# microsoft/ANCE

Measured on NVIDIA H100. Metric: ANN-refresh throughput: passages encoded/sec + queries top-200/sec, 8.8M x 768, higher is better.
Workload: dtype fp16

## Files before the change

### ance_b200/csrc/gemm_core.cuh

```cuda
#pragma once
#include "tc05.cuh"

namespace gemm {

using namespace tc05;

constexpr int BM = 128;
constexpr int BK = 64;
constexpr int MMA_K = 16;

struct WorkShape {
  int M, N, K;
  int num_m_blks;
  int num_n_blks;
  int n_splits;
  int n_blks_per_split;
  unsigned long long hint_a, hint_b;
  int* pace;
  int pace_window;
  int pace_stride;
};

static __device__ __noinline__ void pace_wait(int* pace, int window, int me, int n_clusters, int stride, int seq) {
  volatile int* vp = pace;
  vp[me] = seq;
  const long long t0 = clock64();
  for (;;) {
    int mn = 0x7fffffff;
    for (int c = me % stride; c < n_clusters; c += stride) mn = min(mn, vp[c]);
    if (seq - mn <= window || clock64() - t0 > 200000ll) break;
  }
}

struct EpiCtx {
  int m_blk, split;
  int nb0, nb1;
  int row0;
  int quad;
  int epi_warp;
  int lane;
  int work_seq;
  uint8_t* ep_smem;
};

template <int BN, int STAGES, int CG, int EP_SMEM = 0>
struct SmemPlan {
  static constexpr int kABytes = BM * BK * 2;
  static constexpr int kBBytes = BN * BK * 2;
  static constexpr int kBHalfRows = BN / CG;
  static constexpr int kStageBytes = kABytes + kBBytes;
  static constexpr int kRingBytes = STAGES * kStageBytes;
  static constexpr int kAccPitch = BN + 4;
  static constexpr int kAccOffset = kRingBytes;
  static constexpr int kAccBytes = (BM * kAccPitch * 4 + 1023) / 1024 * 1024;
  static constexpr int kEpOffset = kAccOffset + kAccBytes;
  static constexpr int kBarOffset = kEpOffset + EP_SMEM;
  static constexpr int kBarBytes = (2 * STAGES + 2) * 8;
  static constexpr int kTotal = kBarOffset + kBarBytes;
  static constexpr int kDynamicBytes = kTotal + 1024;
  static_assert(kDynamicBytes <= 232448, "GEMM shared memory exceeds 227 KB");
};

template <uint32_t FMT, int BN>
__device__ __forceinline__ void wgmma_tile(float (&d)[BN / 2], uint64_t adesc, uint64_t bdesc, uint32_t accumulate) {
  if constexpr (BN == 128) wgmma_n128<FMT, 0>(d, adesc, bdesc, accumulate);
  else wgmma_n64<FMT, 0>(d, adesc, bdesc, accumulate);
}

template <class Ep, int BN, int STAGES, int CG, int EPI_WARPS, uint32_t FMT>
__global__ void __launch_bounds__(256 + 32 * EPI_WARPS, 1)
tc05_gemm_kernel(const __grid_constant__ CUtensorMap tmA, const __grid_constant__ CUtensorMap tmB,
                 const WorkShape ws, const __grid_constant__ typename Ep::Params ep) {
  static_assert(BN == 64 || BN == 128, "BN");
  static_assert(CG == 1 || CG == 2, "CG");
  using Plan = SmemPlan<BN, STAGES, CG, Ep::kSmemBytes>;

  extern __shared__ uint8_t smem_raw[];
  uint8_t* smem = reinterpret_cast<uint8_t*>((reinterpret_cast<uintptr_t>(smem_raw) + 1023) & ~uintptr_t(1023));
  float* acc_tile = reinterpret_cast<float*>(smem + Plan::kAccOffset);
  uint64_t* full_bar = reinterpret_cast<uint64_t*>(smem + Plan::kBarOffset);
  uint64_t* empty_bar = full_bar + STAGES;
  uint64_t* afull_bar = empty_bar + STAGES;
  uint64_t* aempty_bar = afull_bar + 1;

  const int warp = threadIdx.x >> 5;
  const int lane = threadIdx.x & 31;
  const uint32_t cta_rank = (CG == 2) ? cluster_ctarank() : 0u;
  const bool leader = (cta_rank == 0);
  const int cluster_id = (CG == 2) ? (blockIdx.x >> 1) : blockIdx.x;
  const int num_clusters = (CG == 2) ? (gridDim.x >> 1) : gridDim.x;
  const int total_work = ws.num_m_blks * ws.n_splits;
  const int num_kb = (ws.K + BK - 1) / BK;

  if (warp == 0 && lane == 0) {
    tma_prefetch_desc(&tmA);
    tma_prefetch_desc(&tmB);
    for (int s = 0; s < STAGES; ++s) {
      mbar_init(&full_bar[s], 1);
      mbar_init(&empty_bar[s], 4 * CG);
    }
    mbar_init(afull_bar, 4);
    mbar_init(aempty_bar, EPI_WARPS);
    fence_barrier_init();
  }
  if constexpr (CG == 2) cluster_sync_all(); else __syncthreads();

  if (warp == 0) {
    if (lane == 0) {
      const uint64_t hint_a = ws.hint_a ? ws.hint_a : Ep::kHintA, hint_b = ws.hint_b ? ws.hint_b : Ep::kHintB;
      Ring<STAGES> ring;
      for (int w = cluster_id; w < total_work; w += num_clusters) {
        const int m_blk = w / ws.n_splits, split = w - m_blk * ws.n_splits;
        const int nb0 = split * ws.n_blks_per_split;
        const int nb1 = min(nb0 + ws.n_blks_per_split, ws.num_n_blks);
        const int a_row = (m_blk * CG + (int)cta_rank) * BM;
        for (int nb = nb0; nb < nb1; ++nb) {
          if (ws.pace != nullptr && leader && ((nb - nb0) & 7) == 0)
            pace_wait(ws.pace, ws.pace_window, cluster_id, num_clusters, ws.pace_stride,
                      ((w - cluster_id) / num_clusters) * ws.num_n_blks + (nb - nb0));
          const int b_row = nb * BN + (int)cta_rank * Plan::kBHalfRows;
          for (int kb = 0; kb < num_kb; ++kb) {
            mbar_wait(&empty_bar[ring.stage], ring.phase ^ 1, 1);
            uint8_t* sa = smem + ring.stage * Plan::kStageBytes;
            uint8_t* sb = sa + Plan::kABytes + cta_rank * (Plan::kBHalfRows * 128);
            mbar_arrive_expect_tx(&full_bar[ring.stage], Plan::kStageBytes);
            tma_load_2d(sa, &tmA, &full_bar[ring.stage], kb * BK, a_row, hint_a);
            if constexpr (CG == 1) tma_load_2d(sb, &tmB, &full_bar[ring.stage], kb * BK, b_row, hint_b);
            else tma_load_2d_multicast(sb, &tmB, &full_bar[ring.stage], kb * BK, b_row, 0x3, hint_b);
            ring.advance();
          }
        }
      }
      if (ws.pace != nullptr && leader) *reinterpret_cast<volatile int*>(ws.pace + cluster_id) = 0x7fffffff;
    }
  } else if (warp >= 4 && warp < 8) {
    Ring<STAGES> ring;
    uint32_t acc_phase = 0;
    auto release = [&](int stage) {
      __syncwarp();
      if (lane == 0) {
        mbar_arrive(&empty_bar[stage]);
        if constexpr (CG == 2) mbar_arrive_cluster(&empty_bar[stage], cta_rank ^ 1u);
      }
    };
    for (int w = cluster_id; w < total_work; w += num_clusters) {
      const int m_blk = w / ws.n_splits, split = w - m_blk * ws.n_splits;
      const int nb0 = split * ws.n_blks_per_split;
      const int nb1 = min(nb0 + ws.n_blks_per_split, ws.num_n_blks);
      (void)m_blk;
      for (int nb = nb0; nb < nb1; ++nb) {
        float acc0[BN / 2], acc1[BN / 2];
#pragma unroll
        for (int i = 0; i < BN / 2; ++i) acc0[i] = acc1[i] = 0.f;
        int prev_stage = -1;
        for (int kb = 0; kb < num_kb; ++kb) {
          mbar_wait(&full_bar[ring.stage], ring.phase, 3);
          const uint32_t sa = smem_u32(smem + ring.stage * Plan::kStageBytes);
          const uint32_t sb = sa + Plan::kABytes;
          wgmma_fence();
#pragma unroll
          for (int k = 0; k < BK / MMA_K; ++k) {
            const uint64_t bdesc = make_desc_k_sw128(sb + k * MMA_K * 2);
            wgmma_tile<FMT, BN>(acc0, make_desc_k_sw128(sa + k * MMA_K * 2), bdesc, 1u);
            wgmma_tile<FMT, BN>(acc1, make_desc_k_sw128(sa + 64 * 128 + k * MMA_K * 2), bdesc, 1u);
          }
          wgmma_commit();
          wgmma_wait<1>();
          wgmma_fence_regs(acc0);
          wgmma_fence_regs(acc1);
          if (prev_stage >= 0) release(prev_stage);
          prev_stage = ring.stage;
          ring.advance();
        }
        wgmma_wait<0>();
        wgmma_fence_regs(acc0);
        wgmma_fence_regs(acc1);
        if (prev_stage >= 0) release(prev_stage);
        mbar_wait(aempty_bar, acc_phase ^ 1, 2);
        acc_store_frag(acc_tile, Plan::kAccPitch, 0, 0, acc0);
        acc_store_frag(acc_tile, Plan::kAccPitch, 64, 0, acc1);
        __syncwarp();
        if (lane == 0) mbar_arrive(afull_bar);
        acc_phase ^= 1;
      }
    }
  } else if (warp >= 8) {
    Ep epi;
    EpiCtx cx;
    cx.quad = warp & 3;
    cx.epi_warp = warp - 8;
    cx.lane = lane;
    cx.work_seq = 0;
    cx.ep_smem = smem + Plan::kEpOffset;
    uint32_t acc_phase = 0;
    const uint32_t tacc = smem_u32(acc_tile) / 4u + static_cast<uint32_t>((cx.quad * 32 + lane) * Plan::kAccPitch);
    for (int w = cluster_id; w < total_work; w += num_clusters, ++cx.work_seq) {
      cx.m_blk = w / ws.n_splits;
      cx.split = w - cx.m_blk * ws.n_splits;
      cx.nb0 = cx.split * ws.n_blks_per_split;
      cx.nb1 = min(cx.nb0 + ws.n_blks_per_split, ws.num_n_blks);
      cx.row0 = (cx.m_blk * CG + (int)cta_rank) * BM;
      epi.begin_work(ep, ws, cx);
      for (int nb = cx.nb0; nb < cx.nb1; ++nb) {
        mbar_wait(afull_bar, acc_phase, 4);
        epi.tile(ep, ws, cx, tacc, nb);
        __syncwarp();
        if (lane == 0) mbar_arrive(aempty_bar);
        acc_phase ^= 1;
      }
      epi.end_work(ep, ws, cx);
    }
    epi.end_kernel(ep, cx);
  }

  if constexpr (CG == 2) cluster_sync_all();
}

constexpr int kMaxDevices = 64;

inline int current_device() {
  int dev = 0;
  cudaGetDevice(&dev);
  return (dev >= 0 && dev < kMaxDevices) ? dev : 0;
}

inline int sm_count() {
  static int n[kMaxDevices] = {};
  const int dev = current_device();
  if (!n[dev]) cudaDeviceGetAttribute(&n[dev], cudaDevAttrMultiProcessorCount, dev);
  return n[dev];
}

template <class Ep, int BN, int STAGES, int CG, int EPI_WARPS, uint32_t FMT>
cudaError_t launch(const CUtensorMap& tmA, const CUtensorMap& tmB, const WorkShape& ws,
                   const typename Ep::Params& ep, int max_ctas, cudaStream_t stream) {
  using Plan = SmemPlan<BN, STAGES, CG, Ep::kSmemBytes>;
  auto kern = tc05_gemm_kernel<Ep, BN, STAGES, CG, EPI_WARPS, FMT>;
  static bool configured[kMaxDevices] = {};
  const int dev = current_device();
  if (!configured[dev]) {
    cudaError_t e = cudaFuncSetAttribute(kern, cudaFuncAttributeMaxDynamicSharedMemorySize, Plan::kDynamicBytes);
    if (e != cudaSuccess) return e;
    configured[dev] = true;
  }
  const int total = ws.num_m_blks * ws.n_splits;
  int clusters = min(total, (max_ctas > 0 ? max_ctas : sm_count()) / CG);
  if (clusters < 1) clusters = 1;
  cudaLaunchConfig_t cfg = {};
  cfg.gridDim = dim3(clusters * CG);
  cfg.blockDim = dim3(256 + 32 * EPI_WARPS);
  cfg.dynamicSmemBytes = Plan::kDynamicBytes;
  cfg.stream = stream;
  cudaLaunchAttribute attr[1];
  attr[0].id = cudaLaunchAttributeClusterDimension;
  attr[0].val.clusterDim.x = CG;
  attr[0].val.clusterDim.y = 1;
  attr[0].val.clusterDim.z = 1;
  cfg.attrs = attr;
  cfg.numAttrs = 1;
  return cudaLaunchKernelEx(&cfg, kern, tmA, tmB, ws, ep);
}

inline WorkShape make_shape(int M, int N, int K, int BN, int CG, int n_splits ) {
  WorkShape ws;
  ws.M = M;
  ws.N = N;
  ws.K = K;
  ws.num_m_blks = (M + BM * CG - 1) / (BM * CG);
  ws.num_n_blks = (N + BN - 1) / BN;
  if (n_splits <= 0 || n_splits > ws.num_n_blks) n_splits = ws.num_n_blks;
  ws.n_blks_per_split = (ws.num_n_blks + n_splits - 1) / n_splits;
  ws.n_splits = (ws.num_n_blks + ws.n_blks_per_split - 1) / ws.n_blks_per_split;
  ws.hint_a = ws.hint_b = 0;
  ws.pace = nullptr;
  ws.pace_window = 0;
  ws.pace_stride = 1;
  return ws;
}

}
```

### ance_b200/csrc/gemm_store.cuh

```cuda
#pragma once
#include "act16.cuh"
#include "gemm_core.cuh"

namespace gemm {

__device__ __forceinline__ float rcp_approx(float x) {
  float r;
  asm("rcp.approx.ftz.f32 %0, %1;" : "=f"(r) : "f"(x));
  return r;
}
__device__ __forceinline__ float ex2_approx(float x) {
  float r;
  asm("ex2.approx.ftz.f32 %0, %1;" : "=f"(r) : "f"(x));
  return r;
}

__device__ __forceinline__ uint64_t pack2(float a, float b) {
  uint64_t r;
  asm("mov.b64 %0, {%1, %2};" : "=l"(r) : "f"(a), "f"(b));
  return r;
}
__device__ __forceinline__ void unpack2(uint64_t v, float& a, float& b) {
  asm("mov.b64 {%0, %1}, %2;" : "=f"(a), "=f"(b) : "l"(v));
}
__device__ __forceinline__ uint64_t fma2(uint64_t a, uint64_t b, uint64_t c) {
  float a0, a1, b0, b1, c0, c1;
  unpack2(a, a0, a1), unpack2(b, b0, b1), unpack2(c, c0, c1);
  return pack2(__fmaf_rn(a0, b0, c0), __fmaf_rn(a1, b1, c1));
}
__device__ __forceinline__ uint64_t mul2(uint64_t a, uint64_t b) {
  float a0, a1, b0, b1;
  unpack2(a, a0, a1), unpack2(b, b0, b1);
  return pack2(__fmul_rn(a0, b0), __fmul_rn(a1, b1));
}

__device__ __forceinline__ void gelu_erf2(float& x0, float& x1) {
  const uint64_t x = pack2(x0, x1);
  const uint64_t ax = x & 0x7FFFFFFF7FFFFFFFull;
  uint64_t p = fma2(pack2(5.38297490e-06f, 5.38297490e-06f), ax, pack2(4.88906371e-05f, 4.88906371e-05f));
  p = fma2(p, ax, pack2(3.80035744e-05f, 3.80035744e-05f));
  p = fma2(p, ax, pack2(3.27762635e-03f, 3.27762635e-03f));
  p = fma2(p, ax, pack2(2.11410057e-02f, 2.11410057e-02f));
  p = fma2(p, ax, pack2(4.98673469e-02f, 4.98673469e-02f));
  p = fma2(p, ax, pack2(1.0f, 1.0f));
  p = mul2(p, p);
  p = mul2(p, p);
  p = mul2(p, p);
  p = mul2(p, p);
  float p0, p1;
  unpack2(p, p0, p1);
  const uint64_t r = pack2(rcp_approx(p0), rcp_approx(p1));
  const uint64_t relu = fma2(ax, pack2(0.5f, 0.5f), mul2(x, pack2(0.5f, 0.5f)));
  unpack2(fma2(mul2(ax, pack2(-0.5f, -0.5f)), r, relu), x0, x1);
}

__device__ __forceinline__ void gelu_logistic2(float& x0, float& x1) {
  const uint64_t x = pack2(x0, x1);
  const uint64_t t = mul2(x, x);
  uint64_t p = fma2(pack2(-3.290565928e-06f, -3.290565928e-06f), t, pack2(8.930850163e-05f, 8.930850163e-05f));
  p = fma2(p, t, pack2(3.548454260e-04f, 3.548454260e-04f));
  p = fma2(p, t, pack2(-1.052178442e-01f, -1.052178442e-01f));
  p = fma2(p, t, pack2(-2.302048445e+00f, -2.302048445e+00f));
  float g0, g1;
  unpack2(mul2(p, x), g0, g1);
  const uint64_t d = fma2(pack2(ex2_approx(g0), ex2_approx(g1)), pack2(1.0f, 1.0f), pack2(1.0f, 1.0f));
  float d0, d1;
  unpack2(d, d0, d1);
  unpack2(mul2(x, pack2(rcp_approx(d0), rcp_approx(d1))), x0, x1);
}

template <int BN, int EPI_WARPS, uint32_t FMT = tc05::kFmtBF16>
struct EpStore {
  using A16 = act16::Act<FMT>;
  static constexpr uint64_t kHintA = tc05::kEvictNormal;
  static constexpr uint64_t kHintB = tc05::kEvictLast;
  static constexpr int kColGroups = EPI_WARPS / 4;
  static constexpr int kColsPerGroup = BN / kColGroups;
  static constexpr int kSlabBytes = BM * 128;
  static constexpr int kSmemBytes = kColGroups * kSlabBytes + 64;
  static_assert(EPI_WARPS % 4 == 0 && kColsPerGroup % 64 == 0, "epilogue warp layout");

  struct alignas(64) Params {
    CUtensorMap tmC;
    CUtensorMap tmR;
    uint16_t* C;
    float* C32;
    const float* bias;
    const uint16_t* R;
    int ldc, ldc32, ldr;
    int act;
  };

  uint32_t rphase;

  __device__ __forceinline__ void begin_work(const Params& p, const WorkShape&, const EpiCtx& cx) {
    if (cx.work_seq == 0 && p.R && p.C && !p.C32) {
      const int cgi = cx.epi_warp >> 2;
      uint64_t* rbar = reinterpret_cast<uint64_t*>(cx.ep_smem + kColGroups * kSlabBytes) + cgi;
      if ((cx.epi_warp & 3) == 0 && cx.lane == 0) {
        tc05::mbar_init(rbar, 1);
        tc05::fence_barrier_init();
      }
      tc05::named_bar_sync(2 + cgi, 128);
      rphase = 0;
    }
  }
  __device__ __forceinline__ void end_work(const Params&, const WorkShape&, const EpiCtx&) {}
  __device__ __forceinline__ void end_kernel(const Params& p, const EpiCtx& cx) {
    if (p.C && (cx.epi_warp & 3) == 0 && cx.lane == 0) tc05::bulk_wait_all();
  }

  __device__ __forceinline__ void finish_chunk(const Params& p, const WorkShape& ws, float (&f)[32], int row,
                                               bool row_ok, int col0, bool direct_residual) {
    const bool full = (col0 + 32 <= ws.N);
    if (p.bias) {
      if (full) {
#pragma unroll
        for (int j = 0; j < 8; ++j) {
          const float4 b = __ldg(reinterpret_cast<const float4*>(p.bias + col0) + j);
          f[j * 4] += b.x; f[j * 4 + 1] += b.y; f[j * 4 + 2] += b.z; f[j * 4 + 3] += b.w;
        }
      } else {
#pragma unroll
        for (int i = 0; i < 32; ++i)
          if (col0 + i < ws.N) f[i] += __ldg(p.bias + col0 + i);
      }
    }
    if (p.act == 1) {
#pragma unroll
      for (int i = 0; i < 32; i += 2) gelu_erf2(f[i], f[i + 1]);
    } else if (p.act == 2) {
#pragma unroll
      for (int i = 0; i < 32; i += 2) gelu_logistic2(f[i], f[i + 1]);
    }
    if (direct_residual && p.R && row_ok) {
      const uint16_t* r = p.R + (size_t)row * p.ldr + col0;
      if (full) {
#pragma unroll
        for (int j = 0; j < 4; ++j) {
          const uint4 q = __ldg(reinterpret_cast<const uint4*>(r) + j);
          const uint32_t h[4] = {q.x, q.y, q.z, q.w};
#pragma unroll
          for (int t = 0; t < 4; ++t) {
            const float2 x = A16::unpack2(h[t]);
            f[j * 8 + t * 2] += x.x;
            f[j * 8 + t * 2 + 1] += x.y;
          }
        }
      } else {
        for (int i = 0; i < 32; ++i)
          if (col0 + i < ws.N) f[i] += A16::to_float(r[i]);
      }
    }
  }

  __device__ __forceinline__ void tile(const Params& p, const WorkShape& ws, const EpiCtx& cx, uint32_t tacc,
                                       int nb) {
    const int cgi = cx.epi_warp >> 2;
    const int r_in_tile = cx.quad * 32 + cx.lane;
    const int row = cx.row0 + r_in_tile;
    const bool row_ok = row < ws.M;
    uint8_t* slab = cx.ep_smem + cgi * kSlabBytes;
    const bool issuer = (cx.epi_warp & 3) == 0 && cx.lane == 0;
#pragma unroll 1
    for (int s = 0; s < kColsPerGroup; s += 64) {
      const int col_in_tile = cgi * kColsPerGroup + s;
      const int col0 = nb * BN + col_in_tile;
      if (col0 >= ws.N) break;
      const bool tma_res = (p.R != nullptr) && (p.C != nullptr) && (p.C32 == nullptr);
      uint64_t* rbar = reinterpret_cast<uint64_t*>(cx.ep_smem + kColGroups * kSlabBytes) + cgi;
      uint8_t* rowp = slab + r_in_tile * 128;
      if (tma_res && issuer) {
        tc05::bulk_wait_read_all();
        tc05::mbar_arrive_expect_tx(rbar, kSlabBytes);
        tc05::tma_load_2d(slab, &p.tmR, rbar, col0, cx.row0, tc05::kEvictFirst);
      }
      constexpr bool kLean = EPI_WARPS > 8;
      uint32_t va[32], vb[kLean ? 1 : 32];
      tc05::acc_ld_x32(tacc + col_in_tile, va);
      if constexpr (!kLean) tc05::acc_ld_x32(tacc + col_in_tile + 32, vb);
      if (!tma_res && p.C) {
        if (issuer) tc05::bulk_wait_read_all();
        tc05::named_bar_sync(2 + cgi, 128);
      }
#pragma unroll
      for (int h = 0; h < 2; ++h) {
        float f[32];
        if constexpr (kLean) {
          if (h == 1) {
            tc05::acc_ld_x32(tacc + col_in_tile + 32, va);
          }
#pragma unroll
          for (int i = 0; i < 32; ++i) f[i] = __uint_as_float(va[i]);
        } else {
#pragma unroll
          for (int i = 0; i < 32; ++i) f[i] = __uint_as_float(h == 0 ? va[i] : vb[i]);
        }
        finish_chunk(p, ws, f, row, row_ok, col0 + h * 32, !tma_res);
        if (p.C32 && row_ok) {
          float* o = p.C32 + (size_t)row * p.ldc32 + col0 + h * 32;
          if (col0 + h * 32 + 32 <= ws.N) {
#pragma unroll
            for (int j = 0; j < 8; ++j)
              reinterpret_cast<float4*>(o)[j] = make_float4(f[j * 4], f[j * 4 + 1], f[j * 4 + 2], f[j * 4 + 3]);
          } else {
            for (int i = 0; i < 32; ++i)
              if (col0 + h * 32 + i < ws.N) o[i] = f[i];
          }
        }
        if (p.C) {
          if (tma_res && h == 0) tc05::mbar_wait(rbar, rphase, 20);
#pragma unroll
          for (int q = 0; q < 4; ++q) {
            uint4* cp = reinterpret_cast<uint4*>(rowp + (((h * 4 + q) ^ (r_in_tile & 7)) * 16));
            if (tma_res) {
              const uint4 rv = *cp;
              const uint32_t rh[4] = {rv.x, rv.y, rv.z, rv.w};
#pragma unroll
              for (int t = 0; t < 4; ++t) {
                const float2 x = A16::unpack2(rh[t]);
                f[q * 8 + t * 2] += x.x;
                f[q * 8 + t * 2 + 1] += x.y;
              }
            }
            uint4 o;
            o.x = A16::pack2(f[q * 8 + 0], f[q * 8 + 1]);
            o.y = A16::pack2(f[q * 8 + 2], f[q * 8 + 3]);
            o.z = A16::pack2(f[q * 8 + 4], f[q * 8 + 5]);
            o.w = A16::pack2(f[q * 8 + 6], f[q * 8 + 7]);
            *cp = o;
          }
        }
      }
      if (p.C) {
        if (tma_res) rphase ^= 1;
        tc05::fence_proxy_async_smem();
        tc05::named_bar_sync(2 + cgi, 128);
        if (issuer) {
          tc05::tma_store_2d(&p.tmC, slab, col0, cx.row0);
          tc05::bulk_commit_group();
        }
      }
    }
  }
};

inline bool make_store_tmap(CUtensorMap* tm, void* C, int M, int N, int ldc) {
  return tc05_host::make_tmap_2d_16b(tm, C, M, N, ldc, BM, 64);
}

}
```

### ance_b200/csrc/search.cu

```cuda
#include <float.h>
#include <math.h>
#include <string.h>

#include <algorithm>
#include <vector>

#include "common.h"
#include "gemm_core.cuh"

namespace {

using namespace tc05;

__host__ __device__ __forceinline__ uint32_t f2ord(float f) {
#ifdef __CUDA_ARCH__
  uint32_t u = __float_as_uint(f);
#else
  uint32_t u;
  memcpy(&u, &f, 4);
#endif
  return u ^ (static_cast<uint32_t>(static_cast<int32_t>(u) >> 31) | 0x80000000u);
}
__host__ __device__ __forceinline__ float ord2f(uint32_t k) {
  uint32_t u = (k & 0x80000000u) ? (k ^ 0x80000000u) : ~k;
#ifdef __CUDA_ARCH__
  return __uint_as_float(u);
#else
  float f;
  memcpy(&f, &u, 4);
  return f;
#endif
}
__device__ __forceinline__ uint64_t make_key(float score, uint32_t row) {
  return (static_cast<uint64_t>(f2ord(score)) << 32) | static_cast<uint64_t>(0xFFFFFFFFu - row);
}
__device__ __forceinline__ float key_score(uint64_t k) { return ord2f(static_cast<uint32_t>(k >> 32)); }
__device__ __forceinline__ uint32_t key_row(uint64_t k) { return 0xFFFFFFFFu - static_cast<uint32_t>(k); }

template <class T>
__device__ __forceinline__ T* shfl_ptr(T* p, int src) {
  uint64_t v = reinterpret_cast<uint64_t>(p);
  uint32_t lo = __shfl_sync(0xffffffffu, static_cast<uint32_t>(v), src);
  uint32_t hi = __shfl_sync(0xffffffffu, static_cast<uint32_t>(v >> 32), src);
  return reinterpret_cast<T*>((static_cast<uint64_t>(hi) << 32) | lo);
}

template <bool kBF16>
__global__ void quantize_rows_kernel(const float* __restrict__ X, uint16_t* __restrict__ X16, int64_t n, int d,
                                     const float* __restrict__ mu, float* __restrict__ norm_hat,
                                     float* __restrict__ norm_delta, unsigned int* __restrict__ max_stats,
                                     int* __restrict__ err_flag) {
  const int lane = threadIdx.x & 31;
  const int64_t row = static_cast<int64_t>(blockIdx.x) * (blockDim.x >> 5) + (threadIdx.x >> 5);
  if (row >= n) return;
  const float* x = X + row * d;
  uint16_t* o = X16 + row * d;
  float sh = 0.f, sd = 0.f, sx = 0.f;
  bool bad = false;
  for (int i = lane * 4; i < d; i += 128) {
    float4 v = __ldg(reinterpret_cast<const float4*>(x + i));
    if (mu) {
      const float4 m = __ldg(reinterpret_cast<const float4*>(mu + i));
      v.x -= m.x; v.y -= m.y; v.z -= m.z; v.w -= m.w;
    }
    float a[4] = {v.x, v.y, v.z, v.w};
    uint16_t q[4];
#pragma unroll
    for (int t = 0; t < 4; ++t) {
      float back;
      if (kBF16) {
        __nv_bfloat16 h = __float2bfloat16_rn(a[t]);
        q[t] = __bfloat16_as_ushort(h);
        back = __bfloat162float(h);
      } else {
        __half h = __float2half_rn(a[t]);
        q[t] = __half_as_ushort(h);
        back = __half2float(h);
      }
      if (!(fabsf(back) <= 3.0e38f)) bad = true;
      sh = fmaf(back, back, sh);
      const float e = a[t] - back;
      sd = fmaf(e, e, sd);
      sx = fmaf(a[t], a[t], sx);
    }
    uint2 pk;
    pk.x = static_cast<uint32_t>(q[0]) | (static_cast<uint32_t>(q[1]) << 16);
    pk.y = static_cast<uint32_t>(q[2]) | (static_cast<uint32_t>(q[3]) << 16);
    *reinterpret_cast<uint2*>(o + i) = pk;
  }
#pragma unroll
  for (int s = 16; s > 0; s >>= 1) {
    sh += __shfl_xor_sync(0xffffffffu, sh, s);
    sd += __shfl_xor_sync(0xffffffffu, sd, s);
    sx += __shfl_xor_sync(0xffffffffu, sx, s);
  }
  if (__any_sync(0xffffffffu, bad) && lane == 0 && err_flag) atomicExch(err_flag, 1);
  if (lane == 0) {
    const float nh = sqrtf(sh) * 1.00001f, nd = (sqrtf(sd) + (mu ? 1.2e-7f * sqrtf(sx) : 0.f)) * 1.00001f;
    if (norm_hat) norm_hat[row] = nh;
    if (norm_delta) norm_delta[row] = nd;
    if (max_stats) {
      atomicMax(&max_stats[0], __float_as_uint(nh));
      atomicMax(&max_stats[1], __float_as_uint(nd));
    }
  }
}

__global__ void __launch_bounds__(256) column_sum_kernel(const float* __restrict__ X, int64_t n, int d, int slab,
                                                         double* __restrict__ sums) {
  const int64_t r0 = static_cast<int64_t>(blockIdx.x) * slab, r1 = min(n, r0 + slab);
  for (int c = threadIdx.x; c < d; c += blockDim.x) {
    double acc = 0.0;
    for (int64_t r = r0; r < r1; ++r) acc += static_cast<double>(__ldg(X + r * d + c));
    atomicAdd(sums + c, acc);
  }
}
__global__ void finalize_mean_kernel(const double* __restrict__ sums, int64_t n, int d, float* __restrict__ mu) {
  const int c = blockIdx.x * blockDim.x + threadIdx.x;
  if (c < d) mu[c] = static_cast<float>(sums[c] / static_cast<double>(n));
}

template <int BN, int CAP, bool kStream = false>
struct EpTopK {
  static constexpr uint64_t kHintA = tc05::kEvictLast;
  static constexpr uint64_t kHintB = tc05::kEvictNormal;
  static constexpr int kEpiWarps = 4;
  static constexpr int kSmemBytes = kStream ? kEpiWarps * 256 * 4 : 0;
  struct Params {
    float* scratch_sc;
    int* scratch_id;
    int* cand_id;
    int* cand_cnt;
    float* cand_thr;
    const float* thr_init;
    int kprime;
    int out_cap;
    int nq, n_rows;
  };

  float thr;
  int cnt;
  float* sc;
  int* id;

  __device__ __forceinline__ void begin_work(const Params& p, const gemm::WorkShape&, const gemm::EpiCtx& cx) {
    const int r = cx.quad * 32 + cx.lane;
    const size_t base = (static_cast<size_t>(blockIdx.x) * gemm::BM + r) * CAP;
    sc = p.scratch_sc + base;
    id = p.scratch_id + base;
    thr = (cx.row0 + r < p.nq) ? (p.thr_init ? __ldg(p.thr_init + cx.row0 + r) : -INFINITY) : INFINITY;
    cnt = 0;
  }

  __device__ __forceinline__ void compact(int kprime, int src, const gemm::EpiCtx& cx) {
    if constexpr (kStream) compact_stream(kprime, src, cx);
    else compact_regs(kprime, src, cx.lane);
  }

  __device__ __forceinline__ void compact_regs(int kprime, int src, int lane) {
    constexpr int kSlots = CAP / 32;
    const int n = __shfl_sync(0xffffffffu, cnt, src);
    float* s_sc = shfl_ptr(sc, src);
    int* s_id = shfl_ptr(id, src);
    uint32_t keys[kSlots];
    int ids[kSlots];
#pragma unroll
    for (int j = 0; j < kSlots; ++j) {
      const int i = j * 32 + lane;
      const bool v = i < n;
      keys[j] = v ? f2ord(s_sc[i]) : 0u;
      ids[j] = v ? s_id[i] : -1;
    }
    uint32_t prefix = 0;
    int remaining = kprime;
#pragma unroll 1
    for (int b = 31; b >= 0; --b) {
      const uint32_t cand = prefix | (1u << b);
      const uint32_t mask = ~((1u << b) - 1u);
      int c = 0;
#pragma unroll
      for (int j = 0; j < kSlots; ++j) c += ((keys[j] & mask) == cand) ? 1 : 0;
      c = __reduce_add_sync(0xffffffffu, c);
      if (c >= remaining) prefix = cand;
      else remaining -= c;
    }
    const uint32_t T = prefix;
    const unsigned lt = (1u << lane) - 1u;
    int base = 0, eq_seen = 0;
#pragma unroll
    for (int j = 0; j < kSlots; ++j) {
      const bool gt = keys[j] > T, eq = keys[j] == T;
      const unsigned eqm = __ballot_sync(0xffffffffu, eq);
      const bool keep = gt || (eq && (eq_seen + __popc(eqm & lt)) < remaining);
      const unsigned km = __ballot_sync(0xffffffffu, keep);
      if (keep) {
        const int pos = base + __popc(km & lt);
        s_sc[pos] = ord2f(keys[j]);
        s_id[pos] = ids[j];
      }
      base += __popc(km);
      eq_seen += __popc(eqm);
    }
    __syncwarp();
    if (lane == src) {
      cnt = kprime;
      thr = ord2f(T);
    }
  }

  __device__ __forceinline__ void compact_stream(int kprime, int src, const gemm::EpiCtx& cx) {
    const int lane = cx.lane;
    const int n = __shfl_sync(0xffffffffu, cnt, src);
    float* s_sc = shfl_ptr(sc, src);
    int* s_id = shfl_ptr(id, src);
    uint32_t* hist = reinterpret_cast<uint32_t*>(cx.ep_smem) + cx.epi_warp * 256;
    uint32_t prefix = 0;
    int remaining = kprime;
#pragma unroll 1
    for (int shift = 24; shift >= 0; shift -= 8) {
      for (int b = lane; b < 256; b += 32) hist[b] = 0u;
      __syncwarp();
      const uint32_t hmask = (shift == 24) ? 0u : ~((1u << (shift + 8)) - 1u);
      for (int i = lane; i < n; i += 32) {
        const uint32_t key = f2ord(s_sc[i]);
        if ((key & hmask) == prefix) atomicAdd(&hist[(key >> shift) & 255u], 1u);
      }
      __syncwarp();
      uint32_t c[8];
      int sum = 0;
#pragma unroll
      for (int j = 0; j < 8; ++j) {
        c[j] = hist[255 - (lane * 8 + j)];
        sum += static_cast<int>(c[j]);
      }
      int incl = sum;
#pragma unroll
      for (int o = 1; o < 32; o <<= 1) {
        const int t = __shfl_up_sync(0xffffffffu, incl, o);
        if (lane >= o) incl += t;
      }
      const int excl = incl - sum;
      const unsigned owner = __ballot_sync(0xffffffffu, excl < remaining && remaining <= incl);
      const int ol = __ffs(owner) - 1;
      int digit = -1, above = 0, acc = excl;
#pragma unroll
      for (int j = 0; j < 8; ++j) {
        if (digit < 0 && acc + static_cast<int>(c[j]) >= remaining) {
          digit = 255 - (lane * 8 + j);
          above = acc;
        }
        acc += static_cast<int>(c[j]);
      }
      digit = __shfl_sync(0xffffffffu, digit, ol);
      above = __shfl_sync(0xffffffffu, above, ol);
      prefix |= static_cast<uint32_t>(digit) << shift;
      remaining -= above;
      __syncwarp();
    }
    const uint32_t T = prefix;
    const unsigned lt = (1u << lane) - 1u;
    int base = 0, eq_seen = 0;
#pragma unroll 1
    for (int i0 = 0; i0 < n; i0 += 32) {
      const int i = i0 + lane;
      const bool v = i < n;
      const float s = v ? s_sc[i] : 0.f;
      const int r = v ? s_id[i] : 0;
      const uint32_t key = f2ord(s);
      const bool gt = v && key > T, eq = v && key == T;
      const unsigned eqm = __ballot_sync(0xffffffffu, eq);
      const bool keep = gt || (eq && (eq_seen + __popc(eqm & lt)) < remaining);
      const unsigned km = __ballot_sync(0xffffffffu, keep);
      __syncwarp();
      if (keep) {
        const int pos = base + __popc(km & lt);
        s_sc[pos] = s;
        s_id[pos] = r;
      }
      base += __popc(km);
      eq_seen += __popc(eqm);
    }
    __syncwarp();
    if (lane == src) {
      cnt = kprime;
      thr = ord2f(T);
    }
  }

  __device__ __forceinline__ void tile(const Params& p, const gemm::WorkShape&, const gemm::EpiCtx& cx,
                                       uint32_t tacc, int nb) {
#pragma unroll 1
    for (int c = 0; c < BN; c += 32) {
      uint32_t v[32];
      acc_ld_x32(tacc + c, v);
      float m = __uint_as_float(v[0]);
#pragma unroll
      for (int i = 1; i < 32; ++i) m = fmaxf(m, __uint_as_float(v[i]));
      if (m > thr) {
        const int col0 = nb * BN + c;
#pragma unroll
        for (int i = 0; i < 32; ++i) {
          const float s = __uint_as_float(v[i]);
          if (s > thr && col0 + i < p.n_rows) {
            sc[cnt] = s;
            id[cnt] = col0 + i;
            ++cnt;
          }
        }
      }
      __syncwarp();
      unsigned need = __ballot_sync(0xffffffffu, cnt > CAP - 32);
      while (need) {
        const int src = __ffs(need) - 1;
        need &= need - 1;
        compact(p.kprime, src, cx);
      }
    }
  }

  __device__ __forceinline__ void end_kernel(const Params&, const gemm::EpiCtx&) {}

  __device__ __forceinline__ void end_work(const Params& p, const gemm::WorkShape& ws, const gemm::EpiCtx& cx) {
    __syncwarp();
    unsigned need = __ballot_sync(0xffffffffu, cnt > p.out_cap);
    while (need) {
      const int src = __ffs(need) - 1;
      need &= need - 1;
      compact(p.kprime, src, cx);
    }
    for (int l = 0; l < 32; ++l) {
      const int row = cx.row0 + cx.quad * 32 + l;
      if (row >= p.nq) break;
      const int n = __shfl_sync(0xffffffffu, cnt, l);
      const float t = __shfl_sync(0xffffffffu, thr, l);
      const int* s_id = shfl_ptr(id, l);
      const size_t slot = static_cast<size_t>(row) * ws.n_splits + cx.split;
      int* out = p.cand_id + slot * p.out_cap;
      for (int i = cx.lane; i < n; i += 32) out[i] = s_id[i];
      if (cx.lane == 0) {
        p.cand_cnt[slot] = n;
        p.cand_thr[slot] = t;
      }
    }
    __syncwarp();
  }
};

template <bool kHost>
__device__ __forceinline__ float4 ld_rows4(const float* p) {
  if constexpr (kHost) {
    float4 v;
    asm("ld.global.v4.f32 {%0, %1, %2, %3}, [%4];" : "=f"(v.x), "=f"(v.y), "=f"(v.z), "=f"(v.w) : "l"(p));
    return v;
  } else {
    return __ldg(reinterpret_cast<const float4*>(p));
  }
}
template <bool kHost>
__device__ __forceinline__ float ld_rows1(const float* p) {
  if constexpr (kHost) {
    float v;
    asm("ld.global.f32 %0, [%1];" : "=f"(v) : "l"(p));
    return v;
  } else {
    return __ldg(p);
  }
}

template <bool kHost = false>
__device__ __forceinline__ double warp_dot_f64(const float* __restrict__ q_smem, const float* __restrict__ p, int d,
                                               int lane) {
  double acc = 0.0;
  if ((d & 127) == 0) {
    for (int i = lane * 4; i < d; i += 128) {
      const float4 a = *reinterpret_cast<const float4*>(q_smem + i);
      const float4 b = ld_rows4<kHost>(p + i);
      acc = fma(static_cast<double>(a.x), static_cast<double>(b.x), acc);
      acc = fma(static_cast<double>(a.y), static_cast<double>(b.y), acc);
      acc = fma(static_cast<double>(a.z), static_cast<double>(b.z), acc);
      acc = fma(static_cast<double>(a.w), static_cast<double>(b.w), acc);
    }
  } else {
    for (int i = lane; i < d; i += 32) acc = fma(static_cast<double>(q_smem[i]), static_cast<double>(ld_rows1<kHost>(p + i)), acc);
  }
#pragma unroll
  for (int s = 16; s > 0; s >>= 1) acc += __shfl_xor_sync(0xffffffffu, acc, s);
  return acc;
}

__device__ __forceinline__ void block_bitonic_desc(uint64_t* keys, int n) {
  for (int size = 2; size <= n; size <<= 1) {
    for (int stride = size >> 1; stride > 0; stride >>= 1) {
      __syncthreads();
      for (int t = threadIdx.x; t < (n >> 1); t += blockDim.x) {
        const int lo = 2 * t - (t & (stride - 1));
        const int hi = lo + stride;
        const bool desc = ((lo & size) == 0);
        const uint64_t a = keys[lo], b = keys[hi];
        if ((a < b) == desc) {
          keys[lo] = b;
          keys[hi] = a;
        }
      }
    }
  }
  __syncthreads();
}

__host__ __device__ inline int next_pow2(int v) {
  int p = 1;
  while (p < v) p <<= 1;
  return p;
}

struct RescoreParams {
  const float* Q;
  const float* P;
  int d;
  const int* cand_id;
  const int* cand_cnt;
  const float* cand_thr;
  int n_splits, cand_stride, k;
  const float* qn_hat;
  const float* qn_delta;
  const unsigned int* pstats;
  const float* mu;
  float accum_rel;
  float* D;
  int64_t* I;
// ... 1174 lines not shown
```

### ance_b200/csrc/tc05.cuh

```cuda
#pragma once

#include <cuda.h>
#include <cuda_bf16.h>
#include <cuda_fp16.h>
#include <cuda_runtime.h>
#include <stdint.h>
#include <stdio.h>

namespace tc05 {

__device__ __forceinline__ uint32_t smem_u32(const void* p) {
  return static_cast<uint32_t>(__cvta_generic_to_shared(p));
}

__device__ __forceinline__ uint32_t cluster_ctarank() {
  uint32_t r;
  asm volatile("mov.u32 %0, %%cluster_ctarank;" : "=r"(r));
  return r;
}

__device__ __forceinline__ void cluster_sync_all() {
  asm volatile("barrier.cluster.arrive.release.aligned;\n" ::: "memory");
  asm volatile("barrier.cluster.wait.acquire.aligned;\n" ::: "memory");
}

constexpr uint64_t kEvictNormal = 0x1000000000000000ull;
constexpr uint64_t kEvictFirst  = 0x12F0000000000000ull;
constexpr uint64_t kEvictLast   = 0x14F0000000000000ull;

__device__ __forceinline__ void mbar_init(uint64_t* bar, uint32_t count) {
  asm volatile("mbarrier.init.shared::cta.b64 [%0], %1;" ::"r"(smem_u32(bar)), "r"(count) : "memory");
}

__device__ __forceinline__ void fence_barrier_init() {
  asm volatile("fence.mbarrier_init.release.cluster;" ::: "memory");
}

__device__ __forceinline__ void fence_proxy_async_smem() {
  asm volatile("fence.proxy.async.shared::cta;" ::: "memory");
}

__device__ __forceinline__ void mbar_arrive_expect_tx(uint64_t* bar, uint32_t bytes) {
  asm volatile("mbarrier.arrive.expect_tx.shared::cta.b64 _, [%0], %1;" ::"r"(smem_u32(bar)), "r"(bytes)
               : "memory");
}

__device__ __forceinline__ void mbar_arrive(uint64_t* bar) {
  asm volatile("mbarrier.arrive.shared::cta.b64 _, [%0];" ::"r"(smem_u32(bar)) : "memory");
}

__device__ __forceinline__ void mbar_arrive_cluster(uint64_t* bar, uint32_t cta) {
  uint32_t remote;
  asm volatile("mapa.shared::cluster.u32 %0, %1, %2;" : "=r"(remote) : "r"(smem_u32(bar)), "r"(cta));
  asm volatile("mbarrier.arrive.release.cluster.shared::cluster.b64 _, [%0];" ::"r"(remote) : "memory");
}

__device__ __forceinline__ uint32_t mbar_try_wait(uint64_t* bar, uint32_t parity) {
  uint32_t ok;
  asm volatile(
      "{\n\t"
      ".reg .pred p;\n\t"
      "mbarrier.try_wait.parity.shared::cta.b64 p, [%1], %2;\n\t"
      "selp.u32 %0, 1, 0, p;\n\t"
      "}"
      : "=r"(ok)
      : "r"(smem_u32(bar)), "r"(parity)
      : "memory");
  return ok;
}

#ifndef TC05_WATCHDOG_CYCLES
#define TC05_WATCHDOG_CYCLES 8000000000ll
#endif
__device__ __forceinline__ void mbar_wait(uint64_t* bar, uint32_t parity, int tag = 0) {
  (void)tag;
  if (mbar_try_wait(bar, parity)) return;
  long long t0 = clock64();
  uint32_t spins = 0;
  while (!mbar_try_wait(bar, parity)) {
    if ((++spins & 0x3FFu) == 0 && clock64() - t0 > TC05_WATCHDOG_CYCLES) asm volatile("trap;");
  }
}

__device__ __forceinline__ void tma_prefetch_desc(const CUtensorMap* tm) {
  asm volatile("prefetch.tensormap [%0];" ::"l"(reinterpret_cast<uint64_t>(tm)) : "memory");
}

__device__ __forceinline__ void tma_load_2d(void* smem_dst, const CUtensorMap* tm, uint64_t* bar, int c0,
                                            int c1, uint64_t hint) {
  asm volatile(
      "cp.async.bulk.tensor.2d.shared::cluster.global.mbarrier::complete_tx::bytes.L2::cache_hint"
      " [%0], [%1, {%3, %4}], [%2], %5;"
      :
      : "r"(smem_u32(smem_dst)), "l"(reinterpret_cast<uint64_t>(tm)), "r"(smem_u32(bar)), "r"(c0), "r"(c1),
        "l"(hint)
      : "memory");
}

__device__ __forceinline__ void tma_load_2d_multicast(void* smem_dst, const CUtensorMap* tm, uint64_t* bar, int c0,
                                                      int c1, uint16_t cta_mask, uint64_t hint) {
  asm volatile(
      "cp.async.bulk.tensor.2d.shared::cluster.global.mbarrier::complete_tx::bytes.multicast::cluster.L2::cache_hint"
      " [%0], [%1, {%3, %4}], [%2], %5, %6;"
      :
      : "r"(smem_u32(smem_dst)), "l"(reinterpret_cast<uint64_t>(tm)), "r"(smem_u32(bar)), "r"(c0), "r"(c1),
        "h"(cta_mask), "l"(hint)
      : "memory");
}

__device__ __forceinline__ void tma_store_2d(const CUtensorMap* tm, const void* smem_src, int c0, int c1) {
  asm volatile("cp.async.bulk.tensor.2d.global.shared::cta.bulk_group [%0, {%2, %3}], [%1];"
               :
               : "l"(reinterpret_cast<uint64_t>(tm)), "r"(smem_u32(smem_src)), "r"(c0), "r"(c1)
               : "memory");
}
__device__ __forceinline__ void bulk_commit_group() { asm volatile("cp.async.bulk.commit_group;" ::: "memory"); }
__device__ __forceinline__ void bulk_wait_read_all() { asm volatile("cp.async.bulk.wait_group.read 0;" ::: "memory"); }
__device__ __forceinline__ void bulk_wait_all() { asm volatile("cp.async.bulk.wait_group 0;" ::: "memory"); }

__device__ __forceinline__ void named_bar_sync(int id, int threads) {
  asm volatile("bar.sync %0, %1;" ::"r"(id), "r"(threads) : "memory");
}

__device__ __forceinline__ uint64_t make_desc_k_sw128(uint32_t smem_addr) {
  uint64_t d = 0;
  d |= static_cast<uint64_t>((smem_addr & 0x3FFFFu) >> 4);
  d |= static_cast<uint64_t>(1) << 16;
  d |= static_cast<uint64_t>(1024 >> 4) << 32;
  d |= static_cast<uint64_t>(1) << 62;
  return d;
}

__device__ __forceinline__ uint64_t make_desc_mn_sw128(uint32_t smem_addr, uint32_t lbo_bytes,
                                                       uint32_t sbo_bytes) {
  uint64_t d = 0;
  d |= static_cast<uint64_t>((smem_addr & 0x3FFFFu) >> 4);
  d |= static_cast<uint64_t>((lbo_bytes >> 4) & 0x3FFFu) << 16;
  d |= static_cast<uint64_t>((sbo_bytes >> 4) & 0x3FFFu) << 32;
  d |= static_cast<uint64_t>(1) << 62;
  return d;
}

enum : uint32_t { kFmtF16 = 0, kFmtBF16 = 1 };

__device__ __forceinline__ void wgmma_fence() { asm volatile("wgmma.fence.sync.aligned;" ::: "memory"); }
__device__ __forceinline__ void wgmma_commit() { asm volatile("wgmma.commit_group.sync.aligned;" ::: "memory"); }
template <int N>
__device__ __forceinline__ void wgmma_wait() { asm volatile("wgmma.wait_group.sync.aligned %0;" ::"n"(N) : "memory"); }
template <int R>
__device__ __forceinline__ void wgmma_fence_regs(float (&d)[R]) {
#pragma unroll
  for (int i = 0; i < R; ++i) asm volatile("" : "+f"(d[i])::"memory");
}

#define TC05_R8(i) "+f"(d[i]), "+f"(d[i + 1]), "+f"(d[i + 2]), "+f"(d[i + 3]), "+f"(d[i + 4]), "+f"(d[i + 5]), "+f"(d[i + 6]), "+f"(d[i + 7])
#define TC05_R32 TC05_R8(0), TC05_R8(8), TC05_R8(16), TC05_R8(24)
#define TC05_R64 TC05_R32, TC05_R8(32), TC05_R8(40), TC05_R8(48), TC05_R8(56)
#define TC05_S32                                                                  \
  "%0, %1, %2, %3, %4, %5, %6, %7, %8, %9, %10, %11, %12, %13, %14, %15, "        \
  "%16, %17, %18, %19, %20, %21, %22, %23, %24, %25, %26, %27, %28, %29, %30, %31"
#define TC05_S64                                                                  \
  TC05_S32 ", "                                                                   \
  "%32, %33, %34, %35, %36, %37, %38, %39, %40, %41, %42, %43, %44, %45, %46, %47, " \
  "%48, %49, %50, %51, %52, %53, %54, %55, %56, %57, %58, %59, %60, %61, %62, %63"
#define TC05_WGMMA(NAME, INSTR, NR, SLIST, RLIST, IA, IB, IP, IT)                                                     \
  template <int kTransB>                                                                                              \
  __device__ __forceinline__ void NAME(float (&d)[NR], uint64_t adesc, uint64_t bdesc, uint32_t accumulate) {        \
    asm volatile("{\n\t.reg .pred p;\n\tsetp.ne.b32 p, %" IP ", 0;\n\t" INSTR " {" SLIST "}, %" IA ", %" IB           \
                 ", p, 1, 1, 0, %" IT ";\n\t}"                                                                        \
                 : RLIST                                                                                              \
                 : "l"(adesc), "l"(bdesc), "r"(accumulate), "n"(kTransB));                                            \
  }
TC05_WGMMA(wgmma_m64n128k16_bf16, "wgmma.mma_async.sync.aligned.m64n128k16.f32.bf16.bf16", 64, TC05_S64, TC05_R64, "64", "65", "66", "67")
TC05_WGMMA(wgmma_m64n128k16_f16, "wgmma.mma_async.sync.aligned.m64n128k16.f32.f16.f16", 64, TC05_S64, TC05_R64, "64", "65", "66", "67")
TC05_WGMMA(wgmma_m64n64k16_bf16, "wgmma.mma_async.sync.aligned.m64n64k16.f32.bf16.bf16", 32, TC05_S32, TC05_R32, "32", "33", "34", "35")
TC05_WGMMA(wgmma_m64n64k16_f16, "wgmma.mma_async.sync.aligned.m64n64k16.f32.f16.f16", 32, TC05_S32, TC05_R32, "32", "33", "34", "35")

template <uint32_t FMT, int kTransB>
__device__ __forceinline__ void wgmma_n128(float (&d)[64], uint64_t adesc, uint64_t bdesc, uint32_t accumulate) {
  if constexpr (FMT == kFmtBF16) wgmma_m64n128k16_bf16<kTransB>(d, adesc, bdesc, accumulate);
  else wgmma_m64n128k16_f16<kTransB>(d, adesc, bdesc, accumulate);
}
template <uint32_t FMT, int kTransB>
__device__ __forceinline__ void wgmma_n64(float (&d)[32], uint64_t adesc, uint64_t bdesc, uint32_t accumulate) {
  if constexpr (FMT == kFmtBF16) wgmma_m64n64k16_bf16<kTransB>(d, adesc, bdesc, accumulate);
  else wgmma_m64n64k16_f16<kTransB>(d, adesc, bdesc, accumulate);
}

template <int R>
__device__ __forceinline__ void acc_store_frag(float* tile, int pitch, int r0, int c0, const float (&d)[R]) {
  const int t = threadIdx.x & 127;
  const int r = r0 + 16 * (t >> 5) + ((t & 31) >> 2);
  const int c = c0 + 2 * (t & 3);
#pragma unroll
  for (int j = 0; j < R / 4; ++j) {
    *reinterpret_cast<float2*>(tile + r * pitch + c + 8 * j) = make_float2(d[4 * j], d[4 * j + 1]);
    *reinterpret_cast<float2*>(tile + (r + 8) * pitch + c + 8 * j) = make_float2(d[4 * j + 2], d[4 * j + 3]);
  }
}

__device__ __forceinline__ void acc_ld_x32(uint32_t waddr, uint32_t* v) {
#pragma unroll
  for (int i = 0; i < 32; i += 4)
    asm volatile("ld.shared.v4.u32 {%0, %1, %2, %3}, [%4];"
                 : "=r"(v[i]), "=r"(v[i + 1]), "=r"(v[i + 2]), "=r"(v[i + 3])
                 : "r"((waddr + i) * 4u)
                 : "memory");
}

template <int kStages>
struct Ring {
  uint32_t stage = 0, phase = 0;
  __device__ __forceinline__ void advance() {
    if (++stage == kStages) {
      stage = 0;
      phase ^= 1;
    }
  }
};

}

namespace tc05_host {

typedef CUresult (*EncodeTiledFn)(CUtensorMap*, CUtensorMapDataType, cuuint32_t, void*, const cuuint64_t*,
                                  const cuuint64_t*, const cuuint32_t*, const cuuint32_t*, CUtensorMapInterleave,
                                  CUtensorMapSwizzle, CUtensorMapL2promotion, CUtensorMapFloatOOBfill);

inline EncodeTiledFn encode_fn() {
  static EncodeTiledFn fn = nullptr;
  if (!fn) {
    void* p = nullptr;
    cudaDriverEntryPointQueryResult q;
    if (cudaGetDriverEntryPoint("cuTensorMapEncodeTiled", &p, cudaEnableDefault, &q) != cudaSuccess ||
        q != cudaDriverEntryPointSuccess)
      return nullptr;
    fn = reinterpret_cast<EncodeTiledFn>(p);
  }
  return fn;
}

inline bool make_tmap_2d_16b(CUtensorMap* tm, const void* base, uint64_t rows, uint64_t cols, uint64_t ld_elems,
                             uint32_t box_rows, uint32_t box_cols = 64) {
  EncodeTiledFn fn = encode_fn();
  if (!fn) return false;
  cuuint64_t gdim[2] = {cols, rows};
  cuuint64_t gstride[1] = {ld_elems * 2};
  cuuint32_t box[2] = {box_cols, box_rows};
  cuuint32_t estr[2] = {1, 1};
  CUresult r = fn(tm, CU_TENSOR_MAP_DATA_TYPE_BFLOAT16, 2, const_cast<void*>(base), gdim, gstride, box, estr,
                  CU_TENSOR_MAP_INTERLEAVE_NONE, CU_TENSOR_MAP_SWIZZLE_128B, CU_TENSOR_MAP_L2_PROMOTION_L2_256B,
                  CU_TENSOR_MAP_FLOAT_OOB_FILL_NONE);
  return r == CUDA_SUCCESS;
}

}
```

Baseline: 17360.

## Add second MMA warpgroup ping-pong for the store GEMM with register rebalancing

Adds an option for two consumer warpgroups that take alternate N tiles, each with its own accumulator-full and accumulator-empty barriers plus a loaded barrier that orders their smem ring use. The producer warpgroup gives up registers via setmaxnreg and the MMA warpgroups gain them. The epilogue alternates between the two sources. The aim is to hide the accumulator store and epilogue handoff of one tile behind the other warpgroup's MMAs. It is enabled only for the store epilogue; search keeps a single warpgroup. Risks are a larger block, register pressure, and a subtle barrier phase protocol, since both warpgroups still share one acc_tile.

After: 17370 (median of 6 runs). Within noise of the previous version (+0.1%).

```diff
diff --git a/ance_b200/csrc/gemm_core.cuh b/ance_b200/csrc/gemm_core.cuh
--- a/ance_b200/csrc/gemm_core.cuh
+++ b/ance_b200/csrc/gemm_core.cuh
@@ -43,7 +43,7 @@
   uint8_t* ep_smem;
 };
 
-template <int BN, int STAGES, int CG, int EP_SMEM = 0>
+template <int BN, int STAGES, int CG, int EP_SMEM = 0, int MMA_WGS = 1>
 struct SmemPlan {
   static constexpr int kABytes = BM * BK * 2;
   static constexpr int kBBytes = BN * BK * 2;
@@ -55,7 +55,7 @@
   static constexpr int kAccBytes = (BM * kAccPitch * 4 + 1023) / 1024 * 1024;
   static constexpr int kEpOffset = kAccOffset + kAccBytes;
   static constexpr int kBarOffset = kEpOffset + EP_SMEM;
-  static constexpr int kBarBytes = (2 * STAGES + 2) * 8;
+  static constexpr int kBarBytes = (2 * STAGES + 2 * MMA_WGS + (MMA_WGS > 1 ? MMA_WGS : 0)) * 8;
   static constexpr int kTotal = kBarOffset + kBarBytes;
   static constexpr int kDynamicBytes = kTotal + 1024;
   static_assert(kDynamicBytes <= 232448, "GEMM shared memory exceeds 227 KB");
@@ -67,13 +67,19 @@
   else wgmma_n64<FMT, 0>(d, adesc, bdesc, accumulate);
 }
 
+template <class Ep, int EPI_WARPS>
+constexpr int kThreads = 128 * (1 + Ep::kMmaWarpgroups) + 32 * EPI_WARPS;
+
 template <class Ep, int BN, int STAGES, int CG, int EPI_WARPS, uint32_t FMT>
-__global__ void __launch_bounds__(256 + 32 * EPI_WARPS, 1)
+__global__ void __launch_bounds__(kThreads<Ep, EPI_WARPS>, 1)
 tc05_gemm_kernel(const __grid_constant__ CUtensorMap tmA, const __grid_constant__ CUtensorMap tmB,
                  const WorkShape ws, const __grid_constant__ typename Ep::Params ep) {
   static_assert(BN == 64 || BN == 128, "BN");
   static_assert(CG == 1 || CG == 2, "CG");
-  using Plan = SmemPlan<BN, STAGES, CG, Ep::kSmemBytes>;
+  constexpr int kMmaWGs = Ep::kMmaWarpgroups;
+  static_assert(kMmaWGs == 1 || (kMmaWGs == 2 && kThreads<Ep, EPI_WARPS> == 512), "MMA warpgroups");
+  constexpr int kEpiWarp0 = 4 + 4 * kMmaWGs;
+  using Plan = SmemPlan<BN, STAGES, CG, Ep::kSmemBytes, kMmaWGs>;
 
   extern __shared__ uint8_t smem_raw[];
   uint8_t* smem = reinterpret_cast<uint8_t*>((reinterpret_cast<uintptr_t>(smem_raw) + 1023) & ~uintptr_t(1023));
@@ -81,14 +87,21 @@
   uint64_t* full_bar = reinterpret_cast<uint64_t*>(smem + Plan::kBarOffset);
   uint64_t* empty_bar = full_bar + STAGES;
   uint64_t* afull_bar = empty_bar + STAGES;
-  uint64_t* aempty_bar = afull_bar + 1;
+  uint64_t* aempty_bar = afull_bar + kMmaWGs;
+  uint64_t* loaded_bar = aempty_bar + kMmaWGs;
 
   const int warp = threadIdx.x >> 5;
   const int lane = threadIdx.x & 31;
-  const uint32_t cta_rank = (CG == 2) ? cluster_ctarank() : 0u;
-  const bool leader = (cta_rank == 0);
-  const int cluster_id = (CG == 2) ? (blockIdx.x >> 1) : blockIdx.x;
-  const int num_clusters = (CG == 2) ? (gridDim.x >> 1) : gridDim.x;
+  uint32_t cta_rank;
+  bool leader;
+  int cluster_id, num_clusters;
+  auto read_grid = [&]() {
+    cta_rank = (CG == 2) ? cluster_ctarank() : 0u;
+    leader = (cta_rank == 0);
+    cluster_id = (CG == 2) ? (blockIdx.x >> 1) : blockIdx.x;
+    num_clusters = (CG == 2) ? (gridDim.x >> 1) : gridDim.x;
+  };
+  if constexpr (kMmaWGs == 1) read_grid();
   const int total_work = ws.num_m_blks * ws.n_splits;
   const int num_kb = (ws.K + BK - 1) / BK;
 
@@ -99,14 +112,21 @@
       mbar_init(&full_bar[s], 1);
       mbar_init(&empty_bar[s], 4 * CG);
     }
-    mbar_init(afull_bar, 4);
-    mbar_init(aempty_bar, EPI_WARPS);
+    for (int j = 0; j < kMmaWGs; ++j) {
+      mbar_init(&afull_bar[j], 4);
+      mbar_init(&aempty_bar[j], EPI_WARPS);
+      if constexpr (kMmaWGs == 2) mbar_init(&loaded_bar[j], 4);
+    }
     fence_barrier_init();
   }
   if constexpr (CG == 2) cluster_sync_all(); else __syncthreads();
 
-  if (warp == 0) {
-    if (lane == 0) {
+  if (kMmaWGs == 2 ? warp < 4 : warp == 0) {
+    if constexpr (kMmaWGs == 2) {
+      setmaxnreg_dec<40>();
+      read_grid();
+    }
+    if (warp == 0 && lane == 0) {
       const uint64_t hint_a = ws.hint_a ? ws.hint_a : Ep::kHintA, hint_b = ws.hint_b ? ws.hint_b : Ep::kHintB;
       Ring<STAGES> ring;
       for (int w = cluster_id; w < total_work; w += num_clusters) {
@@ -133,7 +153,12 @@
       }
       if (ws.pace != nullptr && leader) *reinterpret_cast<volatile int*>(ws.pace + cluster_id) = 0x7fffffff;
     }
-  } else if (warp >= 4 && warp < 8) {
+  } else if (warp >= 4 && warp < kEpiWarp0) {
+    if constexpr (kMmaWGs == 2) {
+      setmaxnreg_inc<168>();
+      read_grid();
+    }
+    const int mma_wg = (kMmaWGs == 2) ? (warp >> 2) - 1 : 0;
     Ring<STAGES> ring;
     uint32_t acc_phase = 0;
     auto release = [&](int stage) {
@@ -143,18 +168,29 @@
         if constexpr (CG == 2) mbar_arrive_cluster(&empty_bar[stage], cta_rank ^ 1u);
       }
     };
+    int seq = 0;
     for (int w = cluster_id; w < total_work; w += num_clusters) {
       const int m_blk = w / ws.n_splits, split = w - m_blk * ws.n_splits;
       const int nb0 = split * ws.n_blks_per_split;
       const int nb1 = min(nb0 + ws.n_blks_per_split, ws.num_n_blks);
       (void)m_blk;
       for (int nb = nb0; nb < nb1; ++nb) {
+        if constexpr (kMmaWGs == 2) {
+          if ((seq++ & 1) != mma_wg) {
+            ring.skip(num_kb);
+            continue;
+          }
+          mbar_wait(&loaded_bar[mma_wg ^ 1], acc_phase ^ (mma_wg == 0 ? 1u : 0u), 5);
+        }
         float acc0[BN / 2], acc1[BN / 2];
 #pragma unroll
         for (int i = 0; i < BN / 2; ++i) acc0[i] = acc1[i] = 0.f;
         int prev_stage = -1;
         for (int kb = 0; kb < num_kb; ++kb) {
           mbar_wait(&full_bar[ring.stage], ring.phase, 3);
+          if constexpr (kMmaWGs == 2) {
+            if (kb == num_kb - 1 && lane == 0) mbar_arrive(&loaded_bar[mma_wg]);
+          }
           const uint32_t sa = smem_u32(smem + ring.stage * Plan::kStageBytes);
           const uint32_t sb = sa + Plan::kABytes;
           wgmma_fence();
@@ -176,23 +212,26 @@
         wgmma_fence_regs(acc0);
         wgmma_fence_regs(acc1);
         if (prev_stage >= 0) release(prev_stage);
-        mbar_wait(aempty_bar, acc_phase ^ 1, 2);
+        mbar_wait(&aempty_bar[mma_wg], acc_phase ^ (mma_wg == 0 ? 1u : 0u), 2);
         acc_store_frag(acc_tile, Plan::kAccPitch, 0, 0, acc0);
         acc_store_frag(acc_tile, Plan::kAccPitch, 64, 0, acc1);
         __syncwarp();
-        if (lane == 0) mbar_arrive(afull_bar);
+        if (lane == 0) mbar_arrive(&afull_bar[mma_wg]);
         acc_phase ^= 1;
       }
     }
-  } else if (warp >= 8) {
+    (void)seq;
+  } else if (warp >= kEpiWarp0) {
+    if constexpr (kMmaWGs == 2) read_grid();
     Ep epi;
     EpiCtx cx;
     cx.quad = warp & 3;
-    cx.epi_warp = warp - 8;
+    cx.epi_warp = warp - kEpiWarp0;
     cx.lane = lane;
     cx.work_seq = 0;
     cx.ep_smem = smem + Plan::kEpOffset;
     uint32_t acc_phase = 0;
+    int src = 0;
     const uint32_t tacc = smem_u32(acc_tile) / 4u + static_cast<uint32_t>((cx.quad * 32 + lane) * Plan::kAccPitch);
     for (int w = cluster_id; w < total_work; w += num_clusters, ++cx.work_seq) {
       cx.m_blk = w / ws.n_splits;
@@ -202,11 +241,17 @@
       cx.row0 = (cx.m_blk * CG + (int)cta_rank) * BM;
       epi.begin_work(ep, ws, cx);
       for (int nb = cx.nb0; nb < cx.nb1; ++nb) {
-        mbar_wait(afull_bar, acc_phase, 4);
+        mbar_wait(&afull_bar[src], acc_phase, 4);
         epi.tile(ep, ws, cx, tacc, nb);
         __syncwarp();
-        if (lane == 0) mbar_arrive(aempty_bar);
-        acc_phase ^= 1;
+        if constexpr (kMmaWGs == 2) {
+          if (lane == 0) mbar_arrive(&aempty_bar[src ^ 1]);
+          src ^= 1;
+          if (src == 0) acc_phase ^= 1;
+        } else {
+          if (lane == 0) mbar_arrive(aempty_bar);
+          acc_phase ^= 1;
+        }
       }
       epi.end_work(ep, ws, cx);
     }
@@ -234,7 +279,7 @@
 template <class Ep, int BN, int STAGES, int CG, int EPI_WARPS, uint32_t FMT>
 cudaError_t launch(const CUtensorMap& tmA, const CUtensorMap& tmB, const WorkShape& ws,
                    const typename Ep::Params& ep, int max_ctas, cudaStream_t stream) {
-  using Plan = SmemPlan<BN, STAGES, CG, Ep::kSmemBytes>;
+  using Plan = SmemPlan<BN, STAGES, CG, Ep::kSmemBytes, Ep::kMmaWarpgroups>;
   auto kern = tc05_gemm_kernel<Ep, BN, STAGES, CG, EPI_WARPS, FMT>;
   static bool configured[kMaxDevices] = {};
   const int dev = current_device();
@@ -248,7 +293,7 @@
   if (clusters < 1) clusters = 1;
   cudaLaunchConfig_t cfg = {};
   cfg.gridDim = dim3(clusters * CG);
-  cfg.blockDim = dim3(256 + 32 * EPI_WARPS);
+  cfg.blockDim = dim3(kThreads<Ep, EPI_WARPS>);
   cfg.dynamicSmemBytes = Plan::kDynamicBytes;
   cfg.stream = stream;
   cudaLaunchAttribute attr[1];
diff --git a/ance_b200/csrc/gemm_store.cuh b/ance_b200/csrc/gemm_store.cuh
--- a/ance_b200/csrc/gemm_store.cuh
+++ b/ance_b200/csrc/gemm_store.cuh
@@ -74,6 +74,7 @@
   using A16 = act16::Act<FMT>;
   static constexpr uint64_t kHintA = tc05::kEvictNormal;
   static constexpr uint64_t kHintB = tc05::kEvictLast;
+  static constexpr int kMmaWarpgroups = 2;
   static constexpr int kColGroups = EPI_WARPS / 4;
   static constexpr int kColsPerGroup = BN / kColGroups;
   static constexpr int kSlabBytes = BM * 128;
diff --git a/ance_b200/csrc/search.cu b/ance_b200/csrc/search.cu
--- a/ance_b200/csrc/search.cu
+++ b/ance_b200/csrc/search.cu
@@ -125,6 +125,7 @@
   static constexpr uint64_t kHintA = tc05::kEvictLast;
   static constexpr uint64_t kHintB = tc05::kEvictNormal;
   static constexpr int kEpiWarps = 4;
+  static constexpr int kMmaWarpgroups = 1;
   static constexpr int kSmemBytes = kStream ? kEpiWarps * 256 * 4 : 0;
   struct Params {
     float* scratch_sc;
diff --git a/ance_b200/csrc/tc05.cuh b/ance_b200/csrc/tc05.cuh
--- a/ance_b200/csrc/tc05.cuh
+++ b/ance_b200/csrc/tc05.cuh
@@ -120,6 +120,17 @@
 
 __device__ __forceinline__ void named_bar_sync(int id, int threads) {
   asm volatile("bar.sync %0, %1;" ::"r"(id), "r"(threads) : "memory");
+}
+
+template <int N>
+__device__ __forceinline__ void setmaxnreg_inc() {
+  static_assert(N % 8 == 0 && N >= 24 && N <= 256, "setmaxnreg");
+  asm volatile("setmaxnreg.inc.sync.aligned.u32 %0;" ::"n"(N));
+}
+template <int N>
+__device__ __forceinline__ void setmaxnreg_dec() {
+  static_assert(N % 8 == 0 && N >= 24 && N <= 256, "setmaxnreg");
+  asm volatile("setmaxnreg.dec.sync.aligned.u32 %0;" ::"n"(N));
 }
 
 __device__ __forceinline__ uint64_t make_desc_k_sw128(uint32_t smem_addr) {
@@ -217,6 +228,11 @@
       phase ^= 1;
     }
   }
+  __device__ __forceinline__ void skip(uint32_t n) {
+    const uint32_t s = stage + n;
+    stage = s % kStages;
+    phase ^= (s / kStages) & 1u;
+  }
 };
 
 }
```
